# terryye/cuda_FlashAttention

Hardware: AMD Instinct MI355X
Metric: FA2 fwd+bwd TFLOP/s at (B=4,H=16,N=8192,d=128); % MFMA peak (higher is better)
Workload: dtype bf16; 1 GPU; FA2 forward+backward bf16, (B=4,H=16,N=8192,d=128) per GPU, non-causal (BASELINE configs[2]); flops = 14 B H N^2 d; B=4, H=16, N=8192, d=128, parallelism=head-sharded replicas x1

## Files before the change

### cuda_flashattention_amd/csrc/fa2_bwd_fused.hip

```cpp
#include <cstdlib>
#include <cstring>
#include <type_traits>

#include "fa2_regfile.h"
#include "fa2_launch.h"

namespace fa2 {

#include "fa2_bwd_fused_body.inc"

typedef __attribute__((address_space(3))) void* fused_lptr_t;

#ifndef FA2_FUSED_DSKEY
#define FA2_FUSED_DSKEY(row) (((row) >> 1) & 7)
#endif

#ifndef FA2_FUSED_DIAG
#define FA2_FUSED_DIAG 0
#endif

constexpr int kFusedRegFile = RF512;

#define FA2_FUSED_CLOBBERS "memory", "vcc", FA2_RF512
#define FA2_FUSED_OPS_128 [r0] "v"(roff[0]), [r1] "v"(roff[1]), [r2] "v"(roff[2]), [r3] "v"(roff[3]), [r4] "v"(roff[4]), [r5] "v"(roff[5]),  \
    [r6] "v"(roff[6]), [r7] "v"(roff[7]), [t0] "v"(toff[0]), [t1] "v"(toff[1]), [t2] "v"(toff[2]), [t3] "v"(toff[3]), [t4] "v"(toff[4]),   \
    [t5] "v"(toff[5]), [t6] "v"(toff[6]), [t7] "v"(toff[7]), [rc] "v"(rcv), [c2] "s"(c2)
#define FA2_FUSED_OPS_64 [r0] "v"(roff[0]), [r1] "v"(roff[1]), [r2] "v"(roff[2]), [r3] "v"(roff[3]), [t0] "v"(toff[0]), [t1] "v"(toff[1]),    \
    [t2] "v"(toff[2]), [t3] "v"(toff[3]), [rc] "v"(rcv), [c2] "s"(c2)

struct FusedStep {
    __amdgpu_buffer_rsrc_t drs, lrs, qrs, grs, rcrs, ctl;
    uint32_t dso, lso, qso, rcso, pvo, mso;
    int need, pval;
};
#define FA2_FUSED_STEP(TEXT, DD, ...)                                                                                                 \
    asm volatile(TEXT                                                                                                                 \
                 : [err] "+s"(err)                                                                                                    \
                 : FA2_FUSED_OPS_##DD, [vm] "i"(VMW), [dqv] "v"(dqv), [drs] "s"(f.drs), [dso] "s"(f.dso), [lrs] "s"(f.lrs), [lso] "s"(f.lso), \
                   [mw] "s"(mw), [mw2] "s"(mw2), [qrs] "s"(f.qrs), [grs] "s"(f.grs), [rcrs] "s"(f.rcrs), [qso] "s"(f.qso),               \
                   [rcso] "s"(f.rcso), [dvo] "v"(dvo), [rcvo] "v"(rcvo), [wv] "s"(wv), [ctl] "s"(f.ctl), [pvo] "s"(f.pvo),               \
                   [mso] "s"(f.mso), [need] "s"(f.need), [pval] "s"(f.pval) __VA_ARGS__                                                \
                 : FA2_FUSED_CLOBBERS, "s12", "s13", "scc", "exec", "m0", "v39")
template <int D, int BUF, int PAR, int VMW, bool MASKED>
__device__ __forceinline__ void fused_cbody(const uint32_t (&roff)[D / 16], const uint32_t (&toff)[D / 16], uint32_t rcv, float c2, uint32_t dqv,
                                            uint32_t dvo, uint32_t rcvo, uint32_t mw, uint32_t mw2, int wv, const FusedStep& f, int& err,
                                            int lo0 = 0, int lo1 = 0)
{
// ... 60 lines not shown

struct FusedArgs {
    BwdArgs b;
    float* dQacc;
    int* ctl;
    int npad;
    const float* rc;
    int fault;
};

#ifdef FA2_TEST_HOOKS
static int g_hook_fault = 0, g_hook_grid = 0, g_hook_last_grid = 0;
extern "C" void fa2_test_set_fused_hooks(int fault, int grid) { g_hook_fault = fault; g_hook_grid = grid; }
extern "C" int fa2_test_last_fused_grid(void) { return g_hook_last_grid; }
#define FA2_HOOK_NOTE_GRID(n) (g_hook_last_grid = (n))
#else
constexpr int g_hook_fault = 0, g_hook_grid = 0;
#define FA2_HOOK_NOTE_GRID(n) ((void)0)
#endif

__device__ __forceinline__ int fused_ctl_ints(int BH, int ncb) { return kCtlHeadmap + 16 * (BH + kHmPad) + 9 * BH * ncb; }

__device__ __forceinline__ int fused_load_sc1(const int* p)
{
    int v;
    asm volatile("global_load_dword %0, %1, off sc1\n\ts_waitcnt vmcnt(0)" : "=v"(v) : "v"(p) : "memory");
    return v;
}
__device__ __forceinline__ void fused_seen_set(int v)
{
    asm volatile("v_mov_b32 v39, %0" : : "s"(v) : "v39");
}

__device__ __forceinline__ int fused_lane_id() { return (int)__builtin_amdgcn_mbcnt_hi(~0u, __builtin_amdgcn_mbcnt_lo(~0u, 0u)); }
template <int OFF>
__device__ __forceinline__ int fused_mail_read(uint32_t lds_addr)
{
    int v;
    asm volatile("v_mov_b32 %0, %1\n\tds_read_b32 %0, %0 offset:%c2\n\ts_waitcnt lgkmcnt(0)" : "=&v"(v) : "s"(lds_addr), "i"(OFF) : "memory");
    return __builtin_amdgcn_readfirstlane(v);
}

__device__ __forceinline__ void fused_store_flag(int* p, int v)
{
    asm volatile("global_store_dword %0, %1, off" : : "v"(p), "v"(v) : "memory");
}

__device__ __forceinline__ bool fused_spin_over(int* ctl, int spins)
{
    if (spins > kSpinLimit) {
        atomicExch(ctl + kCtlError, 1);
        return true;
    }
    return (spins & 1023) == 0 && fused_load_sc1(ctl + kCtlError) != 0;
}

template <bool CHAIN, bool CAUSAL, bool RAGGED = false, bool RECT = false, int HD = 128>
__global__ void __launch_bounds__(256, 1) __attribute__((amdgpu_num_vgpr(39))) fa2_bwd_fused_kernel(FusedArgs fp)
{
    static_assert(CHAIN || !RAGGED, "the atomics form has no ragged variant");
    static_assert(!RECT || (CHAIN && !CAUSAL && !RAGGED), "rectangular blocks: chained, unmasked, aligned");
    static_assert(HD == 128 || (HD == 64 && CHAIN && !RECT), "head_dim 64: chained, square");
    extern __shared__ __attribute__((aligned(16))) char smem[];
    const BwdArgs& p = fp.b;
    constexpr int D = HD, ROWB = 2 * D, KS = D / 16, DT = D / 32;
    constexpr int DQW = 128;
    constexpr int TROWS = 32;
// ... 33 lines not shown
#pragma unroll
    for (int dt = 0; dt < DT; ++dt)
#pragma unroll
        for (int jj = 0; jj < 2; ++jj)
            toff[2 * dt + jj] = lbase + QRING + lds_off<D>(8 * jj + 4 * h + trq, 4 * dt + 2 * trcb + (trp >> 1)) + 8 * (trp & 1);
    const uint32_t rcv = lbase + QRING + 2 * TROWS * ROWB + 16 * h;
    static_for<KS>([&](auto S) {
        constexpr int sidx = decltype(S)::value;
        vset<kFusedRegFile, CL_TOP, ROFFK + sidx>(lbase + lds_off<D>(ki + 64 * wave, 2 * sidx + h));
    });
    const int ecol = W ? wave : (wave & 1), ekey0 = W ? 0 : 128 * (wave >> 1);
    static_for<2>([&](auto JJ) {
        constexpr int jj = decltype(JJ)::value;
        vset<kFusedRegFile, CL_TOP, KT + jj>(lbase + ekey0 * ROWB + lds_off<D>(8 * jj + 4 * h + trq, 4 * ecol + 2 * trcb + (trp >> 1)) + 8 * (trp & 1));
        const int row = 8 * jj + 4 * h + trq;
        vset<kFusedRegFile, CL_TOP, DSRD + jj>(lbase + DSB + (ekey0 + row) * 64 + 8 * ((4 * trcb + trp) ^ FA2_FUSED_DSKEY(row)));
    });
    static_for<4>([&](auto C) {
        constexpr int c = decltype(C)::value;
        vset<kFusedRegFile, CL_TOP, DSWR + c>(lbase + DSB + (64 * wave + ki) * 64 + 8 * (((2 * c) | h) ^ FA2_FUSED_DSKEY(ki)));
    });
    const int doff = lds_dma_off<D>(wave * RPI, lane);
    const uint32_t dqv = CHAIN ? (uint32_t)(wave * 4096 + lane * 16) : (uint32_t)(((4 * h) * D + 32 * wave + ki) * 4);
    const auto rc_rsrc = __builtin_amdgcn_make_buffer_rsrc((void*)fp.rc, 0, (int)(2 * rc_plane * 4), 0x00020000);

    int xcc = 0;
    if constexpr (CHAIN) {
        asm volatile("s_getreg_b32 %0, hwreg(HW_REG_XCC_ID, 0, 4)" : "=s"(xcc));
    }
    int* const prog_base = fp.ctl + kCtlHeadmap + 16 * (p.BH + kHmPad);
#ifndef FA2_FUSED_CAUSAL_G
#define FA2_FUSED_CAUSAL_G 2
#endif
    const int G = CAUSAL ? max(1, min(FA2_FUSED_CAUSAL_G, p.BH / 8)) : 1;
    const auto ctl_rsrc = __builtin_amdgcn_make_buffer_rsrc((void*)fp.ctl, 0, CHAIN ? fused_ctl_ints(p.BH, ncb) * 4 : 0, 0x00020000);

    auto take_ticket = [&]() {
        if (wave == 0 && fused_lane_id() == 0) {
            int hd, j = 0;
            do {
                const int u = atomicAdd(fp.ctl + kCtlTicket + 32 * xcc, 1);
                const int r = u % (G * ncb);
                const int k = (u / (G * ncb)) * G + r % G;
                j = r / G;
                hd = -2;
                if (k < p.BH + kHmPad) {
                    int* hm = fp.ctl + kCtlHeadmap + xcc * (p.BH + kHmPad) + k;
                    int v = 0, spins = 0;
                    if (j == 0) {
                        if (k > 0)
                            while ((v = fused_load_sc1(hm - 1)) == 0)
                                if (fused_spin_over(fp.ctl, ++spins)) break;
                        if (k > 0 && v == 0) {
                            v = -1;
                        } else {
                            const int g = atomicAdd(fp.ctl + kCtlNextHead, 1);
                            v = g < p.BH ? g + 1 : -1;
                        }
                        fused_store_flag(hm, v);
                    } else {
                        while ((v = fused_load_sc1(hm)) == 0)
                            if (fused_spin_over(fp.ctl, ++spins)) { v = -1; break; }
                    }
                    hd = v > 0 ? v - 1 : (r % G == 0 ? -2 : -1);
                }
            } while (hd == -1);
            mail[0] = hd;
            mail[1] = j;
            mail[2] = hd >= 0 ? fused_load_sc1(fp.ctl + kCtlError) : 0;
        }
    };
    auto issue_unit_loads = [&](int head_, int cb_) {
        const size_t slab_ = (size_t)(head_ / p.kv_group) * KHS * ROWB;
        const char* Kh_ = (const char*)p.K + slab_;
        const char* Vh_ = (const char*)p.V + slab_;
        const int kw0_ = cb_ * 256 + wave * 64;
        const int lane_u = (int)__builtin_amdgcn_mbcnt_hi(~0u, __builtin_amdgcn_mbcnt_lo(~0u, 0u));
        const int vk0 = RAGGED ? min(kw0_ + (lane_u & 31), N - 1) : kw0_ + (lane_u & 31);
        const int vk1 = RAGGED ? min(kw0_ + 32 + (lane_u & 31), N - 1) : kw0_ + 32 + (lane_u & 31);
        const char* v0 = Vh_ + (size_t)vk0 * ROWB + 16 * (lane_u >> 5);
        const char* v1 = Vh_ + (size_t)vk1 * ROWB + 16 * (lane_u >> 5);
        static_for<KS>([&](auto S) { fused_load_vfrag<VF, KS, decltype(S)::value>(v0, v1); });
        const auto k_rsrc = __builtin_amdgcn_make_buffer_rsrc((void*)Kh_, 0, N * ROWB, 0x00020000);
#pragma unroll
        for (int j = wave; j < 256 / RPI; j += 4)
            __builtin_amdgcn_raw_ptr_buffer_load_lds(k_rsrc, (fused_lptr_t)(smem + j * 1024), 16, doff, (cb_ * 256 + j * RPI) * ROWB, 0, FA2_FUSED_KV_AUX);
    };

    auto next_unit_loads = [&]() {
        if constexpr (CHAIN) {
            take_ticket();
            __syncthreads();
            const int hn = fused_mail_read<0>(mail_addr);
            if (hn >= 0) issue_unit_loads(hn, fused_mail_read<4>(mail_addr));
        }
    };
    next_unit_loads();

    for (;;) {
#ifdef FA2_FUSED_STATS
        const uint64_t s_pull = __builtin_readcyclecounter();
#endif
        int head, cb, err0 = 0;
        if constexpr (CHAIN) {
            head = fused_mail_read<0>(mail_addr);
            cb = fused_mail_read<4>(mail_addr);
            err0 = fused_mail_read<8>(mail_addr);
            if (head < 0) break;
        } else {
            map_block(blockIdx.x, p.BH, ncb, head, cb);
// ... 19 lines not shown
                const int soff = (t * TROWS + piece * RPI) * ROWB;
                __builtin_amdgcn_raw_ptr_buffer_load_lds(which ? g_rsrc : q_rsrc, (fused_lptr_t)(b + which * (TROWS * ROWB) + piece * 1024),
                                                         16, doff, soff, 0, 0);
            }
            if (wave < 2 && fused_lane_id() < 32)
                __builtin_amdgcn_raw_ptr_buffer_load_lds(rc_rsrc, (fused_lptr_t)(b + 2 * TROWS * ROWB + wave * 128), 4, rcoff, t * TROWS * 4, 0, 0);
        };
        const int n_u = CAUSAL ? ntiles - 8 * cb : ntiles;
        const int niter_u = CAUSAL ? ((n_u + 1 + 5) / 6) * 6 : niter;
        const bool ragged_unit = RAGGED && !CAUSAL && cb == ncb - 1;
        const int first_masked = CAUSAL ? ((n_u - 8) / 6) * 6 : (ragged_unit ? 0 : niter_u);
        auto tl = [&](int u) { return CAUSAL ? ntiles - 1 - u : u; };
        stage(tl(0), 0);
#ifdef FA2_FUSED_PREFILL
        stage(tl(1), 1);
        stage(tl(2), 2);
#endif
        fused_dq_zero<DQT>();
        asm volatile("s_waitcnt vmcnt(0)" ::: "memory");
        __syncthreads();
        if constexpr (W) asm volatile(FA2_FUSED_PRO : : FA2_FUSED_OPS_128, [vm] "i"(VMW) : FA2_FUSED_CLOBBERS);
        else asm volatile(FA2_FUSED64_PRO : : FA2_FUSED_OPS_64, [vm] "i"(VMW) : FA2_FUSED_CLOBBERS);

        const auto dq_rsrc = __builtin_amdgcn_make_buffer_rsrc((void*)(fp.dQacc + (size_t)head * NPQ * DQW), 0, NPQ * DQW * 4, 0x00020000);
        int* const mine = prog_base + head * ncb + cb;
        const int* const prev = mine - 1;
        const int prev_off = (int)((prev - fp.ctl) * 4);
        const int mine_off = (int)((mine - fp.ctl) * 4);
        if constexpr (CHAIN) fused_seen_set(0);
        int err = err0;
#ifdef FA2_FUSED_STATS
        int st_steps = 0, st_polls = 0, st_cycles = 0;
        const uint64_t u0 = __builtin_readcyclecounter();
#endif

        const auto null_rsrc = __builtin_amdgcn_make_buffer_rsrc((void*)fp.dQacc, 0, 0, 0x00020000);
        const bool hp_unit = cb > 0;
        const auto lrs_unit = hp_unit && !(FA2_FUSED_DIAG & 2) ? dq_rsrc : null_rsrc;
        auto step = [&](auto BUF, auto PAR, auto MASKED, auto FAST_, int t) {
            constexpr int buf = decltype(BUF)::value, par = decltype(PAR)::value;
            constexpr bool masked = decltype(MASKED)::value;
            constexpr bool FAST = decltype(FAST_)::value;
            if constexpr (CHAIN && FAST) {
                FusedStep f;
                f.drs = dq_rsrc;
                f.lrs = lrs_unit;
                f.dso = (uint32_t)(tl(t - 1) * TROWS * DQW * 4);
                f.lso = (uint32_t)(tl(t) * TROWS * DQW * 4);
                f.qrs = q_rsrc; f.grs = g_rsrc; f.rcrs = rc_rsrc; f.ctl = ctl_rsrc;
                f.qso = (uint32_t)(tl(t + 1) * TROWS * ROWB + wave * 1024);
                f.rcso = (uint32_t)(tl(t + 1) * TROWS * 4);
                f.pvo = (uint32_t)prev_off; f.mso = (uint32_t)mine_off;
                f.need = (hp_unit && !err && !(FA2_FUSED_DIAG & 1)) ? t + 1 : (int)0x80000000;
                f.pval = t;
#ifdef FA2_TEST_HOOKS
                if (fp.fault && cb == 1) f.pval = 0;
#endif
                fused_cbody<D, buf, par, VMW, false>(roff, toff, rcv, c2, dqv, (uint32_t)doff, (uint32_t)rcoff, lbase + QRING + wave * 1024,
                                                  lbase + QRING + wave * 128, wave, f, err, 0, 0);
            } else if constexpr (CHAIN) {
                FusedStep f;
                const bool live = t >= 1 && t <= n_u;
                const bool more = t + 1 < n_u;
                const bool has_prev = t < n_u && cb > 0;
                f.drs = live ? dq_rsrc : null_rsrc;
                f.lrs = has_prev && !(FA2_FUSED_DIAG & 2) ? dq_rsrc : null_rsrc;
                f.dso = (uint32_t)__builtin_amdgcn_readfirstlane(tl(t - 1) * TROWS * DQW * 4);
                f.lso = (uint32_t)__builtin_amdgcn_readfirstlane(tl(t) * TROWS * DQW * 4);
                f.qrs = q_rsrc; f.grs = g_rsrc; f.rcrs = rc_rsrc; f.ctl = ctl_rsrc;
                f.qso = more ? (uint32_t)(tl(t + 1) * TROWS * ROWB + wave * 1024) : 0x40000000u;
                f.rcso = more ? (uint32_t)(tl(t + 1) * TROWS * 4) : 0x40000000u;
                f.pvo = (uint32_t)prev_off; f.mso = (uint32_t)mine_off;
                f.need = (has_prev && !err && !(FA2_FUSED_DIAG & 1)) ? t + 1 : (int)0x80000000;
                f.pval = t < n_u ? t : n_u;
#ifdef FA2_TEST_HOOKS
                if (fp.fault && cb == 1) f.pval = 0;
#endif
                int lo0 = 0, lo1 = 0;
                if constexpr (masked) {
                    const int lane_m = (int)__builtin_amdgcn_mbcnt_hi(~0u, __builtin_amdgcn_mbcnt_lo(~0u, 0u));
                    if constexpr (CAUSAL) {
                        lo0 = kw0 + (lane_m & 31) - 4 * (lane_m >> 5) - TROWS * tl(t);
                        lo1 = lo0 + 32;
                    } else {
                        lo0 = kw0 + (lane_m & 31) < N ? -0x40000000 : 0x40000000;
                        lo1 = kw0 + 32 + (lane_m & 31) < N ? -0x40000000 : 0x40000000;
                    }
                }
#ifdef FA2_FUSED_STATS2
                const uint64_t b0 = __builtin_readcyclecounter();
#endif
                fused_cbody<D, buf, par, VMW, masked>(roff, toff, rcv, c2, dqv, (uint32_t)doff, (uint32_t)rcoff, lbase + QRING + wave * 1024,
                                                   lbase + QRING + wave * 128, wave, f, err, lo0, lo1);
#ifdef FA2_FUSED_STATS2
                st_cycles += (int)(__builtin_readcyclecounter() - b0);
#endif
            } else {
                static_assert(W || CHAIN, "head_dim 64: chained form only");
                stage(t + 1, (buf + 1) % 3);
                if constexpr (W) fused_body<buf, par, VMW>(roff, toff, rcv, c2);
#ifndef FA2_FUSED_NO_DQ
                if (t >= 1 && t <= ntiles) fused_dq_atomic<DQT>(dq_rsrc, dqv, (uint32_t)__builtin_amdgcn_readfirstlane((t - 1) * TROWS * D * 4));
#endif
                fused_dq_zero<DQT>();
            }
        };
        auto six = [&](auto MASKED, auto FAST_, int t) {
            step(std::integral_constant<int, 0>{}, std::integral_constant<int, 0>{}, MASKED, FAST_, t);
            step(std::integral_constant<int, 1>{}, std::integral_constant<int, 1>{}, MASKED, FAST_, t + 1);
            step(std::integral_constant<int, 2>{}, std::integral_constant<int, 0>{}, MASKED, FAST_, t + 2);
            step(std::integral_constant<int, 0>{}, std::integral_constant<int, 1>{}, MASKED, FAST_, t + 3);
            step(std::integral_constant<int, 1>{}, std::integral_constant<int, 0>{}, MASKED, FAST_, t + 4);
            step(std::integral_constant<int, 2>{}, std::integral_constant<int, 1>{}, MASKED, FAST_, t + 5);
        };
        const int fast_end = CHAIN ? n_u - 2 : -1;
        {
            const int plain_end = first_masked;
            int t = 0;
            asm volatile("" : "+s"(t));
            if (t < plain_end) { six(std::false_type{}, std::false_type{}, t); t += 6; }
#pragma unroll 1
            for (; t + 5 <= fast_end && t < plain_end; t += 6) six(std::false_type{}, std::true_type{}, t);
#pragma unroll 1
            for (; t < plain_end; t += 6) six(std::false_type{}, std::false_type{}, t);
            if constexpr (CHAIN && (CAUSAL || RAGGED)) {
#pragma unroll 1
                for (; t < niter_u; t += 6) six(std::true_type{}, std::false_type{}, t);
            }
        }
        asm volatile("s_waitcnt vmcnt(0) lgkmcnt(0)" ::: "memory");
        if constexpr (CHAIN)
            if (err && !err0 && wave == 0 && fused_lane_id() == 0) atomicExch(fp.ctl + kCtlError, 1);
#ifdef FA2_FUSED_STATS
        const uint64_t s_loop = __builtin_readcyclecounter();
#endif
        next_unit_loads();

        mfma_acc_settle();
        const int lane_ep = (int)__builtin_amdgcn_mbcnt_hi(~0u, __builtin_amdgcn_mbcnt_lo(~0u, 0u));
        const int ki_ep = lane_ep & 31, h_ep = lane_ep >> 5;
        static_for<2>([&](auto KB) {
            constexpr int kb = decltype(KB)::value;
            const int key = kw0 + 32 * kb + ki_ep;
            const size_t slab_k = RECT ? (size_t)head * KHS * ROWB : slab;
            char* const dKb = (char*)p.dK + slab_k;
            char* const dVb = (char*)p.dV + slab_k;
            const uint32_t koff = (uint32_t)key * ROWB + 16u * h_ep;
            char* dKk = dKb + koff;
            char* dVk = dVb + koff;
            static_for<2 * DT>([&](auto G) {
                constexpr int dt = decltype(G)::value / 2, gp = decltype(G)::value % 2;
                constexpr int RK = 16 * (kb * DT + dt) + 8 * gp, RV = 32 * DT + RK;
                auto pack4 = [&](float a, float b, float c, float d, float sc) {
                    bf16x4 v;
                    v[0] = (__bf16)(a * sc); v[1] = (__bf16)(b * sc); v[2] = (__bf16)(c * sc); v[3] = (__bf16)(d * sc);
                    return __builtin_bit_cast(u32x2, v);
                };
                auto emit = [&](u32x2 x, u32x2 y, char* dst) {
                    const auto s0 = __builtin_amdgcn_permlane32_swap(x[0], y[0], false, false);
                    const auto s1 = __builtin_amdgcn_permlane32_swap(x[1], y[1], false, false);
                    const u32x4 o = {s0[0], s1[0], s0[1], s1[1]};
#ifdef FA2_FUSED_ST_NT
                    if (!RAGGED || key < N) __builtin_nontemporal_store(o, reinterpret_cast<u32x4*>(dst + 2 * (32 * dt + 16 * gp)));
#else
                    if (!RAGGED || key < N) *reinterpret_cast<u32x4*>(dst + 2 * (32 * dt + 16 * gp)) = o;
#endif
                };
                emit(pack4(aread<RK>(), aread<RK + 1>(), aread<RK + 2>(), aread<RK + 3>(), p.scale),
                     pack4(aread<RK + 4>(), aread<RK + 5>(), aread<RK + 6>(), aread<RK + 7>(), p.scale), dKk);
                emit(pack4(aread<RV>(), aread<RV + 1>(), aread<RV + 2>(), aread<RV + 3>(), 1.0f),
                     pack4(aread<RV + 4>(), aread<RV + 5>(), aread<RV + 6>(), aread<RV + 7>(), 1.0f), dVk);
            });
        });
#ifdef FA2_FUSED_STATS
        if (CHAIN && wave == 0 && fused_lane_id() == 0) {
            atomicAdd(fp.ctl + kCtlError + 1, st_steps);
            atomicAdd(fp.ctl + kCtlError + 2, st_polls);
            atomicAdd((unsigned long long*)(fp.ctl + kCtlError + 4), (unsigned long long)st_cycles);
            atomicAdd((unsigned long long*)(fp.ctl + kCtlError + 6), (unsigned long long)(__builtin_readcyclecounter() - u0));
            int* rec = prog_base + p.BH * ncb + 8 * (head * ncb + cb);
            rec[0] = xcc; rec[1] = st_cycles; rec[2] = (int)(u0 - s_pull); rec[3] = (int)(__builtin_readcyclecounter() - s_loop);
            *(unsigned long long*)(rec + 4) = u0; *(unsigned long long*)(rec + 6) = __builtin_readcyclecounter();
        }
#endif
        if constexpr (!CHAIN) break;
    }
}

__global__ void __launch_bounds__(256) fa2_bwd_fused_dq_out_kernel(const float* __restrict__ acc, __bf16* __restrict__ dQ, size_t n8, float scale,
                                                                    const int* __restrict__ err)
{
    const float poison = (err && *err) ? __builtin_nanf("") : 0.0f;
    const size_t stride = (size_t)gridDim.x * 256;
    for (size_t i = (size_t)blockIdx.x * 256 + threadIdx.x; i < n8; i += stride) {
        const f32x4 a = reinterpret_cast<const f32x4*>(acc)[2 * i], b = reinterpret_cast<const f32x4*>(acc)[2 * i + 1];
        bf16x8 o;
#pragma unroll
        for (int e = 0; e < 4; ++e) { o[e] = (__bf16)(a[e] * scale + poison); o[4 + e] = (__bf16)(b[e] * scale + poison); }
        reinterpret_cast<bf16x8*>(dQ)[i] = o;
    }
}

__global__ void __launch_bounds__(256) fa2_bwd_fused_dq_out_chain_kernel(const float* __restrict__ acc, __bf16* __restrict__ dQ, size_t n4, float scale,
                                                                          const int* __restrict__ err, int N, int NP, int qhs)
{
    const float poison = *err ? __builtin_nanf("") : 0.0f;
    const size_t stride = (size_t)gridDim.x * 256;
    const size_t tiles = (size_t)(NP / 32);
    for (size_t i = (size_t)blockIdx.x * 256 + threadIdx.x; i < n4; i += stride) {
        const f32x4 a = reinterpret_cast<const f32x4*>(acc)[i];
        const int lane = (int)(i & 63), g = (int)((i >> 6) & 3), wave = (int)((i >> 8) & 3);
        const size_t tg = i >> 10, head = tg / tiles;
        const int row = (int)(tg % tiles) * 32 + 8 * g + 4 * (lane >> 5);
        __bf16* o = dQ + (head * (size_t)qhs + row) * 128 + 32 * wave + (lane & 31);
#pragma unroll
// ... 182 lines not shown
```

### cuda_flashattention_amd/csrc/fa2_common.h

```cpp
#pragma once
#include <hip/hip_runtime.h>
#include <stdint.h>

#include <type_traits>
#include <utility>

namespace fa2 {

typedef __attribute__((ext_vector_type(8))) __bf16 bf16x8;
typedef __attribute__((ext_vector_type(4))) __bf16 bf16x4;
typedef __attribute__((ext_vector_type(16))) float f32x16;
typedef __attribute__((ext_vector_type(4))) float f32x4;
typedef __attribute__((ext_vector_type(2))) float f32x2;
typedef __attribute__((ext_vector_type(4))) uint32_t u32x4;
typedef __attribute__((ext_vector_type(2))) uint32_t u32x2;

constexpr float kLog2e = 1.4426950408889634f;

template <int D>
__device__ __forceinline__ int lds_off(int row, int ch)
{
    static_assert(D == 64 || D == 128, "head_dim must be 64 or 128");
    if constexpr (D == 128)
        return 256 * row + 16 * (ch ^ (((row & 3) << 2) | ((row >> 2) & 3)));
    else
        return 128 * row + 16 * (ch ^ ((((row >> 1) & 1) << 2) | ((row >> 2) & 3)));
}

template <int D>
__device__ __forceinline__ int lds_dma_off(int row0, int lane)
{
    constexpr int ROWB = 2 * D, CPR = D / 8;
    const int drow = lane / CPR, dslot = lane % CPR, prow = row0 + drow;
    return drow * ROWB + 16 * ((lds_off<D>(prow, dslot) - ROWB * prow) >> 4);
}

template <typename F, int... I>
__device__ __forceinline__ void static_for_impl(F&& f, std::integer_sequence<int, I...>)
{
    (f(std::integral_constant<int, I>{}), ...);
}
template <int N, typename F>
__device__ __forceinline__ void static_for(F&& f)
{
    static_for_impl(f, std::make_integer_sequence<int, N>{});
}

__device__ __forceinline__ float half_max(float x)
{
    const uint32_t u = __float_as_uint(x);
    auto r = __builtin_amdgcn_permlane32_swap(u, u, false, false);
    return fmaxf(__uint_as_float(r[0]), __uint_as_float(r[1]));
}

__device__ __forceinline__ float half_sum(float x)
{
    const uint32_t u = __float_as_uint(x);
    auto r = __builtin_amdgcn_permlane32_swap(u, u, false, false);
    return __uint_as_float(r[0]) + __uint_as_float(r[1]);
}

__device__ __forceinline__ constexpr int acc_row(int r, int h)
{
    return (r & 3) + 8 * (r >> 2) + 4 * h;
}

__device__ __forceinline__ void map_block(int bid, int n_heads, int nrb, int& head, int& rb)
// ... 26 lines not shown
```

### cuda_flashattention_amd/csrc/fa2_fwd1_bf16.hip

```cpp
#include <type_traits>

#include "fa2_fwd_softmax.h"
#include "fa2_launch.h"

namespace fa2 {

#include "fa2_fwd_body.inc"

constexpr int kF1Rows = 256;
constexpr int kF1Bufs = 4;
constexpr float kF1SumLimit = 1.2089258e24f;
constexpr float kF1LiftAt = 1.0737418e9f;
constexpr float kF1LiftBy = 44.3614196f;
enum { F1_PLAIN = 0, F1_MASKED = 1, F1_NOMAX = 2 };

typedef __attribute__((address_space(3))) void* f1_lptr_t;

template <int QBS> constexpr int kF1RegFile = QBS == 2 ? RF512 : RF128;

struct F1Dma {
    __amdgpu_buffer_rsrc_t krs, vrs;
    uint32_t mw, dvo, kso;
};

template <int D, int QBS, int BUF, int KB, int MODE>
__device__ __forceinline__ void f1_body(float c2, int& need, const int (&hi)[2], const F1Dma& dma)
{
#define FA2_F1_CASE(TAG, DD, QQ, B, K, MV, M)                                                                                      \
    if constexpr (D == DD && QBS == QQ && BUF == B && KB == K && MODE == MV)                                                         \
        FA2_RF_ASM(kF1RegFile<QQ>, CL_ORDER, FA2_FWD_BODY_##TAG##_B##B##_K##K##_##M, [need] "=&s"(need),                                                     \
                   [c2] "s"(c2) FA2_COMMA [hi0] "v"(hi[0]) FA2_COMMA [hi1] "v"(hi[1]) FA2_COMMA [ninf] "v"(-INFINITY)           \
                       FA2_COMMA [mw] "s"(dma.mw) FA2_COMMA [dvo] "v"(dma.dvo) FA2_COMMA [krs] "s"(dma.krs)                     \
                       FA2_COMMA [vrs] "s"(dma.vrs) FA2_COMMA [kso] "s"(dma.kso));
#define FA2_F1_CASES_B(TAG, DD, QQ, K, MV, M) \
    FA2_F1_CASE(TAG, DD, QQ, 0, K, MV, M) FA2_F1_CASE(TAG, DD, QQ, 1, K, MV, M) FA2_F1_CASE(TAG, DD, QQ, 2, K, MV, M) FA2_F1_CASE(TAG, DD, QQ, 3, K, MV, M)
#define FA2_F1_CASES_V(TAG, DD, QQ, K) \
    FA2_F1_CASES_B(TAG, DD, QQ, K, F1_PLAIN, M0) FA2_F1_CASES_B(TAG, DD, QQ, K, F1_MASKED, M1) FA2_F1_CASES_B(TAG, DD, QQ, K, F1_NOMAX, X)
    FA2_F1_CASES_V(D128Q2, 128, 2, 0) FA2_F1_CASES_V(D128Q2, 128, 2, 1)
    FA2_F1_CASES_V(D64Q2, 64, 2, 0) FA2_F1_CASES_V(D64Q2, 64, 2, 1) FA2_F1_CASES_V(D64Q2, 64, 2, 2) FA2_F1_CASES_V(D64Q2, 64, 2, 3)
    FA2_F1_CASES_V(D64Q1, 64, 1, 0) FA2_F1_CASES_V(D64Q1, 64, 1, 1) FA2_F1_CASES_V(D64Q1, 64, 1, 2) FA2_F1_CASES_V(D64Q1, 64, 1, 3)
#undef FA2_F1_CASES_V
#undef FA2_F1_CASES_B
#undef FA2_F1_CASE
}

template <int D, int QBS>
__device__ __forceinline__ void f1_prologue()
{
    if constexpr (D == 128) FA2_RF_ASM(RF512, CL_ORDER, FA2_FWD_PRO_D128Q2, , );
// ... 227 lines not shown
            constexpr int kb = decltype(KB_)::value;
            const int j = t * NH + kb;
            int need = 0;
            if constexpr (GENERAL) {
                if (j >= JB) return;
                const int key0 = j * 32;
                bool masked = key0 + 32 > Nk;
                if (CAUSAL) masked = masked || key0 + 31 > q0 + p.causal_shift;
                if (masked) {
                    int hi[2] = {0, 0};
#pragma unroll
                    for (int qb = 0; qb < QBS; ++qb) hi[qb] = (CAUSAL ? min(Nk, qrow[qb] + p.causal_shift + 1) : Nk) - key0 - 4 * h;
                    f1_body<D, QBS, B, kb, F1_MASKED>(c2, need, hi, dma);
                } else {
                    const int hi[2] = {0, 0};
                    f1_body<D, QBS, B, kb, F1_PLAIN>(c2, need, hi, dma);
                }
            } else {
                const int hi[2] = {0, 0};
                f1_body<D, QBS, B, kb, FAST>(c2, need, hi, dma);
            }
            if (__builtin_amdgcn_readfirstlane(need | (int)have_pend)) update(need);
        });
    };
    const int ntl = (JB + NH - 1) / NH;
    int nfull = Nk / KV;
    if (CAUSAL) nfull = min(nfull, max(0, (q0 + p.causal_shift + 1) / KV));
    nfull = min(nfull, J / NH) & ~3;
    int nfull_wg = Nk / KV;
    if (CAUSAL) nfull_wg = min(nfull_wg, max(0, (rb * kF1Rows + (kF1Waves - 1) * WROWS + p.causal_shift + 1) / KV));
    nfull_wg = min(nfull_wg, J / NH) & ~3;
    using I0 = Int<0>; using I1 = Int<1>; using I2 = Int<2>; using I3 = Int<3>;
    int* const redo_flag = reinterpret_cast<int*>(smem + 2 * KRING);
    bool safe = false;
    for (;;) {
        init_pass();
        out_of_range = false;
        asm volatile("s_waitcnt vmcnt(0)" ::: "memory");
        __syncthreads();
        f1_prologue<D, QBS>();
        int t = 0;
        for (; t < nfull; t += 4) {
            if (safe) {
                run_tile(I0{}, I0{}, t); run_tile(I1{}, I0{}, t + 1); run_tile(I2{}, I0{}, t + 2); run_tile(I3{}, I0{}, t + 3);
            } else if (t == 0) {
                run_tile(I0{}, I0{}, t); run_tile(I1{}, I2{}, t + 1); run_tile(I2{}, I2{}, t + 2); run_tile(I3{}, I2{}, t + 3);
            } else {
                lift();
                run_tile(I0{}, I2{}, t); run_tile(I1{}, I2{}, t + 1); run_tile(I2{}, I2{}, t + 2); run_tile(I3{}, I2{}, t + 3);
            }
        }
        FA2_FWD_TAIL_TILES(run_tile, t, ntl);
        asm volatile("s_waitcnt vmcnt(0) lgkmcnt(0)" ::: "memory");
        if (safe || nfull_wg == 0) break;
        bool bad = out_of_range;
        static_for<QBS>([&](auto QB) {
            constexpr int qb = decltype(QB)::value;
            bad = bad || !(half_sum(vget<ST + 2 * qb>() + vget<ST + 2 * qb + 1>()) < kF1SumLimit);
        });
        if (tid == 0) *redo_flag = 0;
        __syncthreads();
        if (__any(bad) && lane == 0) *redo_flag = 1;
        __syncthreads();
        if (*redo_flag == 0) break;
        asm volatile("; fa2-cold: a row sum left the range of the rounds without maxima: the row block again, with maxima");
        safe = true;
    }
    mfma_acc_settle();
    const bool fin = !STATE || p.finalize;
    static_for<QBS>([&](auto QB) {
        constexpr int qb = decltype(QB)::value;
        const float l_tot = half_sum(vget<ST + 2 * qb>() + vget<ST + 2 * qb + 1>());
        const size_t qoff = (size_t)head * qhs + qrow[qb];
        const float pa = pend[qb];
        const float inv = (fin ? (l_tot > 0.0f ? 1.0f / l_tot : 0.0f) : 1.0f) * pa;
        static_for<2 * DT>([&](auto G) {
            constexpr int dt = decltype(G)::value / 2, gp = decltype(G)::value % 2;
            constexpr int R = A_O + (qb * DT + dt) * 16 + 8 * gp;
            f32x4 v, w;
            fwd_read_o8<R>(inv, v, w);
            if (fin) {
                const u32x4 o = fwd_pack_o8_bf16(v, w);
                if (qrow[qb] < Nq) *reinterpret_cast<u32x4*>((char*)p.O + qoff * ROWB + 2 * (32 * dt + 16 * gp + 8 * h)) = o;
            } else if (qrow[qb] < Nq) {
                *reinterpret_cast<f32x4*>(p.Oacc + qoff * D + 32 * dt + 16 * gp + 4 * h) = v;
                *reinterpret_cast<f32x4*>(p.Oacc + qoff * D + 32 * dt + 16 * gp + 8 + 4 * h) = w;
            }
        });
        if (qrow[qb] < Nq && h == 0) {
            if (fin) {
                p.L[qoff] = m_run[qb] + __builtin_logf(l_tot);
            } else {
                p.L[qoff] = l_tot;
                p.M[qoff] = m_run[qb];
            }
        }
    });
    }
}

template <int D, int QBS, bool CAUSAL, bool STATE>
__device__ __forceinline__ void fwd1_dense_impl(const FwdArgs& p)
{
    const int nrb = (p.Nq + kF1Rows - 1) / kF1Rows;
    const int nwg = (CAUSAL && !STATE) ? (nrb + 1) / 2 : nrb;
    int head, wi;
    map_block(blockIdx.x, p.BH, nwg, head, wi);
    fa2_fwd1_impl<D, QBS, CAUSAL, STATE>(p, head, wi);
}

template <int D, int QBS, bool CAUSAL>
__device__ __forceinline__ void fwd1_varlen_impl(const VarlenFwdArgs& v)
{
    constexpr size_t ROWB = D * 2;
    int head, idx;
    map_block(blockIdx.x, v.a.BH, v.n_items, head, idx);
    const VarlenItem it = uniform_item(v.items, idx);
    FwdArgs p = v.a;
    p.Q = (const char*)p.Q + (size_t)it.q_row0 * ROWB;
    p.O = (char*)p.O + (size_t)it.q_row0 * ROWB;
    p.L += it.q_row0;
    p.K = (const char*)p.K + (size_t)it.k_row0 * ROWB;
    p.V = (const char*)p.V + (size_t)it.k_row0 * ROWB;
    p.Nq = it.len_q; p.Nk = it.len_k;
    p.resume = 0; p.finalize = 1;
    const int nrb = (it.len_q + kF1Rows - 1) / kF1Rows;
    fa2_fwd1_impl<D, QBS, CAUSAL, true>(p, head, CAUSAL ? nrb - 1 - it.block : it.block);
}

template <int D, bool CAUSAL, bool STATE>
// ... 70 lines not shown
```

Measured before the change: 1341 TFLOP/s.

## Stage dK/dV epilogue through LDS for row-contiguous stores; group dense tickets

New measurement: 1320 TFLOP/s. -1.6%, worse.

```diff
diff --git a/cuda_flashattention_amd/csrc/fa2_bwd_fused.hip b/cuda_flashattention_amd/csrc/fa2_bwd_fused.hip
--- a/cuda_flashattention_amd/csrc/fa2_bwd_fused.hip
+++ b/cuda_flashattention_amd/csrc/fa2_bwd_fused.hip
@@ -10,9 +10,20 @@
 #include "fa2_bwd_fused_body.inc"
 
 typedef __attribute__((address_space(3))) void* fused_lptr_t;
+typedef __attribute__((address_space(1))) u32x4 fused_gvec_t;
 
 #ifndef FA2_FUSED_DSKEY
 #define FA2_FUSED_DSKEY(row) (((row) >> 1) & 7)
+#endif
+
+#ifndef FA2_FUSED_ROWST
+#define FA2_FUSED_ROWST 1
+#endif
+#ifndef FA2_FUSED_ROWST_NG
+#define FA2_FUSED_ROWST_NG 2
+#endif
+#ifndef FA2_FUSED_DENSE_G
+#define FA2_FUSED_DENSE_G 2
 #endif
 
 #ifndef FA2_FUSED_DIAG
@@ -239,7 +250,8 @@
 #ifndef FA2_FUSED_CAUSAL_G
 #define FA2_FUSED_CAUSAL_G 2
 #endif
-    const int G = CAUSAL ? max(1, min(FA2_FUSED_CAUSAL_G, p.BH / 8)) : 1;
+    const int G = CAUSAL ? max(1, min(FA2_FUSED_CAUSAL_G, p.BH / 8))
+                         : ((FA2_FUSED_DENSE_G > 1 && CHAIN && !RECT) ? max(1, min(FA2_FUSED_DENSE_G, p.BH / 8)) : 1);
     const auto ctl_rsrc = __builtin_amdgcn_make_buffer_rsrc((void*)fp.ctl, 0, CHAIN ? fused_ctl_ints(p.BH, ncb) * 4 : 0, 0x00020000);
 
     auto take_ticket = [&]() {
@@ -473,6 +485,71 @@
         next_unit_loads();
 
         mfma_acc_settle();
+#if FA2_FUSED_ROWST
+        if constexpr (!CHAIN) __syncthreads();
+        auto lane_fresh = [&]() {
+            int l;
+            asm volatile("v_mbcnt_lo_u32_b32 %0, -1, 0\n\tv_mbcnt_hi_u32_b32 %0, -1, %0" : "=v"(l));
+            return l;
+        };
+        static_for<4>([&](auto B) {
+            constexpr int kb = decltype(B)::value / 2;
+            constexpr bool isv = decltype(B)::value % 2;
+            constexpr int CPRW = ROWB / 16, RPS = 1024 / ROWB;
+            char* const stg = smem + DSB + wave * 8192;
+            const float sc = isv ? 1.0f : p.scale;
+            {
+                const int lw = lane_fresh(), kiw = lw & 31;
+                char* const wrow = stg + kiw * ROWB;
+                const int cw = (lw >> 5) ^ (kiw & 7);
+                static_for<2 * DT>([&](auto G) {
+                    constexpr int dt = decltype(G)::value / 2, gp = decltype(G)::value % 2;
+                    constexpr int R0 = (isv ? 32 * DT : 0) + 16 * (kb * DT + dt) + 8 * gp;
+                    auto pack2 = [&](float a, float b) {
+                        typedef float pair_f32 __attribute__((ext_vector_type(2)));
+                        typedef __bf16 pair_bf16 __attribute__((ext_vector_type(2)));
+                        const pair_f32 v = {a * sc, b * sc};
+                        return __builtin_bit_cast(uint32_t, __builtin_convertvector(v, pair_bf16));
+                    };
+                    auto pack4 = [&](float a, float b, float c, float d) { return u32x2{pack2(a, b), pack2(c, d)}; };
+                    const u32x2 x = pack4(aread<R0>(), aread<R0 + 1>(), aread<R0 + 2>(), aread<R0 + 3>());
+                    const u32x2 y = pack4(aread<R0 + 4>(), aread<R0 + 5>(), aread<R0 + 6>(), aread<R0 + 7>());
+                    const auto s0 = __builtin_amdgcn_permlane32_swap(x[0], y[0], false, false);
+                    const auto s1 = __builtin_amdgcn_permlane32_swap(x[1], y[1], false, false);
+                    const u32x4 o = {s0[0], s1[0], s0[1], s1[1]};
+                    *reinterpret_cast<u32x4*>(wrow + 16 * (cw ^ (4 * dt + 2 * gp))) = o;
+                    __builtin_amdgcn_sched_barrier(0);
+                });
+            }
+            const int key0 = kw0 + 32 * kb;
+            const size_t slab_k = RECT ? (size_t)head * KHS * ROWB : slab;
+            char* const dst = (char*)(isv ? p.dV : p.dK) + slab_k + (size_t)key0 * ROWB;
+            const uint32_t lr = (uint32_t)lane_fresh();
+            const uint32_t loff = 16u * lr;
+            const int rr = (int)(lr / CPRW), cc = (int)(lr % CPRW);
+            constexpr int NG = (W && (CAUSAL || RAGGED)) ? 1 : FA2_FUSED_ROWST_NG;
+            static_for<32 / RPS / NG>([&](auto GR) {
+                constexpr int i0 = decltype(GR)::value * NG;
+                uintptr_t gb = (uintptr_t)dst + 1024 * i0;
+                asm volatile("" : "+s"(gb));
+                u32x4 o[NG];
+                static_for<NG>([&](auto I) {
+                    const int row = RPS * (i0 + decltype(I)::value) + rr;
+                    o[decltype(I)::value] = *reinterpret_cast<const u32x4*>(stg + row * ROWB + 16 * (cc ^ (row & 7)));
+                });
+                static_for<NG>([&](auto I) {
+                    constexpr int i = decltype(I)::value;
+                    const int left = min(N - key0 - RPS * (i0 + i), 32);
+#ifdef FA2_FUSED_ST_NT
+                    if (!RAGGED || (int)loff < left * ROWB) __builtin_nontemporal_store(o[i], (fused_gvec_t*)(gb + (uint32_t)(loff + 1024 * i)));
+#else
+                    if (!RAGGED || (int)loff < left * ROWB) *(fused_gvec_t*)(gb + (uint32_t)(loff + 1024 * i)) = o[i];
+#endif
+                });
+                __builtin_amdgcn_sched_barrier(0);
+            });
+        });
+#else
         const int lane_ep = (int)__builtin_amdgcn_mbcnt_hi(~0u, __builtin_amdgcn_mbcnt_lo(~0u, 0u));
         const int ki_ep = lane_ep & 31, h_ep = lane_ep >> 5;
         static_for<2>([&](auto KB) {
@@ -508,6 +585,7 @@
                      pack4(aread<RV + 4>(), aread<RV + 5>(), aread<RV + 6>(), aread<RV + 7>(), 1.0f), dVk);
             });
         });
+#endif
 #ifdef FA2_FUSED_STATS
         if (CHAIN && wave == 0 && fused_lane_id() == 0) {
             atomicAdd(fp.ctl + kCtlError + 1, st_steps);
```

## Stage dK/dV and O epilogue stores through swizzled LDS for row-contiguous global writes

Applied to the files above, without the earlier changes.

Result: no change. 1276 TFLOP/s before, 1273 TFLOP/s after (-0.2%).

```diff
diff --git a/cuda_flashattention_amd/csrc/fa2_bwd_fused.hip b/cuda_flashattention_amd/csrc/fa2_bwd_fused.hip
--- a/cuda_flashattention_amd/csrc/fa2_bwd_fused.hip
+++ b/cuda_flashattention_amd/csrc/fa2_bwd_fused.hip
@@ -139,7 +139,12 @@
     asm volatile("v_mov_b32 v39, %0" : : "s"(v) : "v39");
 }
 
-__device__ __forceinline__ int fused_lane_id() { return (int)__builtin_amdgcn_mbcnt_hi(~0u, __builtin_amdgcn_mbcnt_lo(~0u, 0u)); }
+__device__ __forceinline__ int fused_lane_id()
+{
+    int l;
+    asm volatile("v_mbcnt_lo_u32_b32 %0, -1, 0\n\tv_mbcnt_hi_u32_b32 %0, -1, %0" : "=v"(l));
+    return l;
+}
 template <int OFF>
 __device__ __forceinline__ int fused_mail_read(uint32_t lds_addr)
 {
@@ -239,16 +244,19 @@
 #ifndef FA2_FUSED_CAUSAL_G
 #define FA2_FUSED_CAUSAL_G 2
 #endif
-    const int G = CAUSAL ? max(1, min(FA2_FUSED_CAUSAL_G, p.BH / 8)) : 1;
+    auto group_of = [](int heads) { return CAUSAL ? max(1, min(FA2_FUSED_CAUSAL_G, heads / 8)) : 1; };
     const auto ctl_rsrc = __builtin_amdgcn_make_buffer_rsrc((void*)fp.ctl, 0, CHAIN ? fused_ctl_ints(p.BH, ncb) * 4 : 0, 0x00020000);
 
     auto take_ticket = [&]() {
         if (wave == 0 && fused_lane_id() == 0) {
             int hd, j = 0;
+            int heads = p.BH, nkb = ncb;
+            asm volatile("" : "+s"(heads), "+s"(nkb));
+            const int G = group_of(heads), gn = G * nkb;
             do {
                 const int u = atomicAdd(fp.ctl + kCtlTicket + 32 * xcc, 1);
-                const int r = u % (G * ncb);
-                const int k = (u / (G * ncb)) * G + r % G;
+                const int r = u % gn;
+                const int k = (u / gn) * G + r % G;
                 j = r / G;
                 hd = -2;
                 if (k < p.BH + kHmPad) {
@@ -282,7 +290,7 @@
         const char* Kh_ = (const char*)p.K + slab_;
         const char* Vh_ = (const char*)p.V + slab_;
         const int kw0_ = cb_ * 256 + wave * 64;
-        const int lane_u = (int)__builtin_amdgcn_mbcnt_hi(~0u, __builtin_amdgcn_mbcnt_lo(~0u, 0u));
+        const int lane_u = fused_lane_id();
         const int vk0 = RAGGED ? min(kw0_ + (lane_u & 31), N - 1) : kw0_ + (lane_u & 31);
         const int vk1 = RAGGED ? min(kw0_ + 32 + (lane_u & 31), N - 1) : kw0_ + 32 + (lane_u & 31);
         const char* v0 = Vh_ + (size_t)vk0 * ROWB + 16 * (lane_u >> 5);
@@ -368,6 +376,7 @@
 #ifdef FA2_FUSED_STATS
         int st_steps = 0, st_polls = 0, st_cycles = 0;
         const uint64_t u0 = __builtin_readcyclecounter();
+        uint64_t s_two = u0;
 #endif
 
         const auto null_rsrc = __builtin_amdgcn_make_buffer_rsrc((void*)fp.dQacc, 0, 0, 0x00020000);
@@ -414,7 +423,7 @@
 #endif
                 int lo0 = 0, lo1 = 0;
                 if constexpr (masked) {
-                    const int lane_m = (int)__builtin_amdgcn_mbcnt_hi(~0u, __builtin_amdgcn_mbcnt_lo(~0u, 0u));
+                    const int lane_m = fused_lane_id();
                     if constexpr (CAUSAL) {
                         lo0 = kw0 + (lane_m & 31) - 4 * (lane_m >> 5) - TROWS * tl(t);
                         lo1 = lo0 + 32;
@@ -430,6 +439,9 @@
                                                    lbase + QRING + wave * 128, wave, f, err, lo0, lo1);
 #ifdef FA2_FUSED_STATS2
                 st_cycles += (int)(__builtin_readcyclecounter() - b0);
+#endif
+#ifdef FA2_FUSED_STATS
+                if (t == 1) s_two = __builtin_readcyclecounter();
 #endif
             } else {
                 static_assert(W || CHAIN, "head_dim 64: chained form only");
@@ -471,42 +483,76 @@
         const uint64_t s_loop = __builtin_readcyclecounter();
 #endif
         next_unit_loads();
+#ifdef FA2_FUSED_STATS
+        const uint64_t s_next = __builtin_readcyclecounter();
+#endif
 
         mfma_acc_settle();
-        const int lane_ep = (int)__builtin_amdgcn_mbcnt_hi(~0u, __builtin_amdgcn_mbcnt_lo(~0u, 0u));
+        const int lane_ep = fused_lane_id();
         const int ki_ep = lane_ep & 31, h_ep = lane_ep >> 5;
+        static_assert(32 * ROWB <= 2 * (FA2_FUSED_DSTILE / 4) && FA2_FUSED_DSTILE == FA2_FUSED64_DSTILE, "the wave's rows of the two dS tiles hold a block");
+        constexpr int DSWAVE = FA2_FUSED_DSTILE / 4;
+        constexpr int HOP = FA2_FUSED_DSTILE - DSWAVE;
+        constexpr int EPI_PER = W ? 2 : 1;
+        static_assert(epi_read_periodic<D, EPI_PER>(), "the rows of reads i and i + EPI_PER have the same swizzle key");
+        const uint32_t img = lbase + DSB + wave * DSWAVE;
+        const uint32_t wrow = img + ROWB * ki_ep + (W ? (ki_ep >> 4) * HOP : 0);
+        uint32_t wkey = 16 * (h_ep ^ (ki_ep & 7));
+        uint32_t rd[EPI_PER];
+#pragma unroll
+        for (int k = 0; k < EPI_PER; ++k) rd[k] = img + epi_read_off<D>(lane_ep, k) - 1024 * k;
         static_for<2>([&](auto KB) {
             constexpr int kb = decltype(KB)::value;
-            const int key = kw0 + 32 * kb + ki_ep;
+            const int key0 = kw0 + 32 * kb;
             const size_t slab_k = RECT ? (size_t)head * KHS * ROWB : slab;
-            char* const dKb = (char*)p.dK + slab_k;
-            char* const dVb = (char*)p.dV + slab_k;
-            const uint32_t koff = (uint32_t)key * ROWB + 16u * h_ep;
-            char* dKk = dKb + koff;
-            char* dVk = dVb + koff;
+            char* const dKb = (char*)p.dK + slab_k + (size_t)key0 * ROWB;
+            char* const dVb = (char*)p.dV + slab_k + (size_t)key0 * ROWB;
+            auto pack4 = [&](float a, float b, float c, float d, float sc) {
+                bf16x4 v;
+                v[0] = (__bf16)(a * sc); v[1] = (__bf16)(b * sc); v[2] = (__bf16)(c * sc); v[3] = (__bf16)(d * sc);
+                return __builtin_bit_cast(u32x2, v);
+            };
+            auto put = [&](u32x2 x, u32x2 y, int g, char* dst) {
+                if (g == 0) asm volatile("" : "+v"(wkey));
+
+                const auto s0 = __builtin_amdgcn_permlane32_swap(x[0], y[0], false, false);
+                const auto s1 = __builtin_amdgcn_permlane32_swap(x[1], y[1], false, false);
+                const u32x4 o = {s0[0], s1[0], s0[1], s1[1]};
+#ifdef FA2_FUSED_EPI_DIRECT
+                if (!RAGGED || key0 + ki_ep < N) *reinterpret_cast<u32x4*>(dst + (uint32_t)ki_ep * ROWB + 32 * g + 16 * h_ep) = o;
+#else
+                *lds_ptr16(wrow + (wkey ^ (32 * g))) = o;
+#endif
+            };
+            auto rows_out = [&](char* dst) {
+#ifndef FA2_FUSED_EPI_DIRECT
+                static_for<NINS>([&](auto I) {
+                    constexpr int i = decltype(I)::value;
+                    const u32x4 o = *lds_ptr16(rd[i % EPI_PER] + 1024 * i + (1024 * i >= DSWAVE ? HOP : 0));
+                    char* const at = dst + 1024 * i + (uint32_t)(16 * lane_ep);
+                    if (!RAGGED || key0 + RPI * i + lane_ep / CPR < N) {
+#ifdef FA2_FUSED_ST_NT
+                        __builtin_nontemporal_store(o, reinterpret_cast<u32x4*>(at));
+#else
+                        *reinterpret_cast<u32x4*>(at) = o;
+#endif
+                    }
+                    if constexpr (i % 2 == 1) asm volatile("" ::: "memory");
+                });
+#endif
+            };
             static_for<2 * DT>([&](auto G) {
-                constexpr int dt = decltype(G)::value / 2, gp = decltype(G)::value % 2;
-                constexpr int RK = 16 * (kb * DT + dt) + 8 * gp, RV = 32 * DT + RK;
-                auto pack4 = [&](float a, float b, float c, float d, float sc) {
-                    bf16x4 v;
-                    v[0] = (__bf16)(a * sc); v[1] = (__bf16)(b * sc); v[2] = (__bf16)(c * sc); v[3] = (__bf16)(d * sc);
-                    return __builtin_bit_cast(u32x2, v);
-                };
-                auto emit = [&](u32x2 x, u32x2 y, char* dst) {
-                    const auto s0 = __builtin_amdgcn_permlane32_swap(x[0], y[0], false, false);
-                    const auto s1 = __builtin_amdgcn_permlane32_swap(x[1], y[1], false, false);
-                    const u32x4 o = {s0[0], s1[0], s0[1], s1[1]};
-#ifdef FA2_FUSED_ST_NT
-                    if (!RAGGED || key < N) __builtin_nontemporal_store(o, reinterpret_cast<u32x4*>(dst + 2 * (32 * dt + 16 * gp)));
-#else
-                    if (!RAGGED || key < N) *reinterpret_cast<u32x4*>(dst + 2 * (32 * dt + 16 * gp)) = o;
-#endif
-                };
-                emit(pack4(aread<RK>(), aread<RK + 1>(), aread<RK + 2>(), aread<RK + 3>(), p.scale),
-                     pack4(aread<RK + 4>(), aread<RK + 5>(), aread<RK + 6>(), aread<RK + 7>(), p.scale), dKk);
-                emit(pack4(aread<RV>(), aread<RV + 1>(), aread<RV + 2>(), aread<RV + 3>(), 1.0f),
-                     pack4(aread<RV + 4>(), aread<RV + 5>(), aread<RV + 6>(), aread<RV + 7>(), 1.0f), dVk);
+                constexpr int g = decltype(G)::value, RK = 16 * kb * DT + 8 * g;
+                put(pack4(aread<RK>(), aread<RK + 1>(), aread<RK + 2>(), aread<RK + 3>(), p.scale),
+                    pack4(aread<RK + 4>(), aread<RK + 5>(), aread<RK + 6>(), aread<RK + 7>(), p.scale), g, dKb);
             });
+            rows_out(dKb);
+            static_for<2 * DT>([&](auto G) {
+                constexpr int g = decltype(G)::value, RV = 32 * DT + 16 * kb * DT + 8 * g;
+                put(pack4(aread<RV>(), aread<RV + 1>(), aread<RV + 2>(), aread<RV + 3>(), 1.0f),
+                    pack4(aread<RV + 4>(), aread<RV + 5>(), aread<RV + 6>(), aread<RV + 7>(), 1.0f), g, dVb);
+            });
+            rows_out(dVb);
         });
 #ifdef FA2_FUSED_STATS
         if (CHAIN && wave == 0 && fused_lane_id() == 0) {
@@ -515,8 +561,14 @@
             atomicAdd((unsigned long long*)(fp.ctl + kCtlError + 4), (unsigned long long)st_cycles);
             atomicAdd((unsigned long long*)(fp.ctl + kCtlError + 6), (unsigned long long)(__builtin_readcyclecounter() - u0));
             int* rec = prog_base + p.BH * ncb + 8 * (head * ncb + cb);
-            rec[0] = xcc; rec[1] = st_cycles; rec[2] = (int)(u0 - s_pull); rec[3] = (int)(__builtin_readcyclecounter() - s_loop);
-            *(unsigned long long*)(rec + 4) = u0; *(unsigned long long*)(rec + 6) = __builtin_readcyclecounter();
+            rec[0] = xcc;
+#ifdef FA2_FUSED_STATS2
+            rec[1] = st_cycles;
+#else
+            rec[1] = (int)(s_next - s_loop);
+#endif
+            rec[2] = (int)(u0 - s_pull); rec[3] = (int)(__builtin_readcyclecounter() - s_loop);
+            *(unsigned long long*)(rec + 4) = u0; rec[6] = (int)(__builtin_readcyclecounter() - u0); rec[7] = (int)(s_two - u0);
         }
 #endif
         if constexpr (!CHAIN) break;
diff --git a/cuda_flashattention_amd/csrc/fa2_common.h b/cuda_flashattention_amd/csrc/fa2_common.h
--- a/cuda_flashattention_amd/csrc/fa2_common.h
+++ b/cuda_flashattention_amd/csrc/fa2_common.h
@@ -33,6 +33,28 @@
     constexpr int ROWB = 2 * D, CPR = D / 8;
     const int drow = lane / CPR, dslot = lane % CPR, prow = row0 + drow;
     return drow * ROWB + 16 * ((lds_off<D>(prow, dslot) - ROWB * prow) >> 4);
+}
+
+template <int D>
+__device__ __forceinline__ constexpr int epi_off(int row, int pc)
+{
+    static_assert(D == 64 || D == 128, "head_dim must be 64 or 128");
+    return 2 * D * row + 16 * (pc ^ (row & 7));
+}
+template <int D>
+__device__ __forceinline__ constexpr int epi_read_off(int lane, int i)
+{
+    return epi_off<D>(lane / (D / 8) + (512 / D) * i, lane % (D / 8));
+}
+typedef __attribute__((address_space(3))) u32x4 lds_u32x4;
+__device__ __forceinline__ lds_u32x4* lds_ptr16(uint32_t addr) { return reinterpret_cast<lds_u32x4*>((uintptr_t)addr); }
+template <int D, int PER>
+constexpr bool epi_read_periodic()
+{
+    for (int l = 0; l < 64; ++l)
+        for (int i = 0; i < D / 16; ++i)
+            if (epi_read_off<D>(l, i) != epi_read_off<D>(l, i % PER) + 1024 * (i - i % PER)) return false;
+    return true;
 }
 
 template <typename F, int... I>
diff --git a/cuda_flashattention_amd/csrc/fa2_fwd1_bf16.hip b/cuda_flashattention_amd/csrc/fa2_fwd1_bf16.hip
--- a/cuda_flashattention_amd/csrc/fa2_fwd1_bf16.hip
+++ b/cuda_flashattention_amd/csrc/fa2_fwd1_bf16.hip
@@ -15,6 +15,22 @@
 enum { F1_PLAIN = 0, F1_MASKED = 1, F1_NOMAX = 2 };
 
 typedef __attribute__((address_space(3))) void* f1_lptr_t;
+
+#ifdef FA2_F1_EPI_STAMPS
+constexpr unsigned kF1StampSlots = 1u << 16;
+__device__ unsigned g_f1_stamps[4 * kF1StampSlots];
+extern "C" __attribute__((visibility("default"))) int fa2_debug_read_fwd_stamps(unsigned* host, int clear)
+{
+    hipError_t e = hipDeviceSynchronize();
+    if (e == hipSuccess) e = hipMemcpyFromSymbol(host, HIP_SYMBOL(g_f1_stamps), sizeof(unsigned) * 4 * kF1StampSlots);
+    if (e == hipSuccess && clear) {
+        void* dev = nullptr;
+        e = hipGetSymbolAddress(&dev, HIP_SYMBOL(g_f1_stamps));
+        if (e == hipSuccess) e = hipMemset(dev, 0, sizeof(unsigned) * 4 * kF1StampSlots);
+    }
+    return (int)e;
+}
+#endif
 
 template <int QBS> constexpr int kF1RegFile = QBS == 2 ? RF512 : RF128;
 
@@ -308,6 +324,10 @@
     nfull_wg = min(nfull_wg, J / NH) & ~3;
     using I0 = Int<0>; using I1 = Int<1>; using I2 = Int<2>; using I3 = Int<3>;
     int* const redo_flag = reinterpret_cast<int*>(smem + 2 * KRING);
+    const bool fin = !STATE || p.finalize;
+#ifdef FA2_F1_EPI_STAMPS
+    const uint64_t s_wg = __builtin_readcyclecounter();
+#endif
     bool safe = false;
     for (;;) {
         init_pass();
@@ -328,7 +348,10 @@
         }
         FA2_FWD_TAIL_TILES(run_tile, t, ntl);
         asm volatile("s_waitcnt vmcnt(0) lgkmcnt(0)" ::: "memory");
-        if (safe || nfull_wg == 0) break;
+        if (safe || nfull_wg == 0) {
+            if (fin) __syncthreads();
+            break;
+        }
         bool bad = out_of_range;
         static_for<QBS>([&](auto QB) {
             constexpr int qb = decltype(QB)::value;
@@ -342,8 +365,20 @@
         asm volatile("; fa2-cold: a row sum left the range of the rounds without maxima: the row block again, with maxima");
         safe = true;
     }
+#ifdef FA2_F1_EPI_STAMPS
+    const uint64_t s_loop = __builtin_readcyclecounter();
+#endif
     mfma_acc_settle();
-    const bool fin = !STATE || p.finalize;
+    static_assert(kF1Rows * ROWB <= KRING, "the K ring holds the workgroup's rows of O");
+    constexpr int EPI_PER = D == 128 ? 2 : 1;
+    static_assert(epi_read_periodic<D, EPI_PER>(), "the rows of reads i and i + EPI_PER have the same swizzle key");
+    int lane_e = lane;
+    asm volatile("" : "+v"(lane_e));
+    const uint32_t img = lbase + wave * QBS * 32 * ROWB;
+    const uint32_t wrow = img + ROWB * (lane_e & 31), wkey = 16 * ((lane_e >> 5) ^ (lane_e & 7));
+    uint32_t rd[EPI_PER];
+#pragma unroll
+    for (int k = 0; k < EPI_PER; ++k) rd[k] = img + epi_read_off<D>(lane_e, k) - 1024 * k;
     static_for<QBS>([&](auto QB) {
         constexpr int qb = decltype(QB)::value;
         const float l_tot = half_sum(vget<ST + 2 * qb>() + vget<ST + 2 * qb + 1>());
@@ -351,18 +386,33 @@
         const float pa = pend[qb];
         const float inv = (fin ? (l_tot > 0.0f ? 1.0f / l_tot : 0.0f) : 1.0f) * pa;
         static_for<2 * DT>([&](auto G) {
-            constexpr int dt = decltype(G)::value / 2, gp = decltype(G)::value % 2;
+            constexpr int g = decltype(G)::value, dt = g / 2, gp = g % 2;
             constexpr int R = A_O + (qb * DT + dt) * 16 + 8 * gp;
             f32x4 v, w;
             fwd_read_o8<R>(inv, v, w);
             if (fin) {
                 const u32x4 o = fwd_pack_o8_bf16(v, w);
+#ifdef FA2_F1_EPI_DIRECT
                 if (qrow[qb] < Nq) *reinterpret_cast<u32x4*>((char*)p.O + qoff * ROWB + 2 * (32 * dt + 16 * gp + 8 * h)) = o;
+#else
+                *lds_ptr16(wrow + qb * 32 * ROWB + (wkey ^ (32 * g))) = o;
+#endif
             } else if (qrow[qb] < Nq) {
                 *reinterpret_cast<f32x4*>(p.Oacc + qoff * D + 32 * dt + 16 * gp + 4 * h) = v;
                 *reinterpret_cast<f32x4*>(p.Oacc + qoff * D + 32 * dt + 16 * gp + 8 + 4 * h) = w;
             }
         });
+#ifndef FA2_F1_EPI_DIRECT
+        if (fin) {
+            const int row0 = q0 + 32 * qb;
+            char* const dst = (char*)p.O + ((size_t)head * qhs + row0) * ROWB + (uint32_t)(16 * lane_e);
+            static_for<32 / RPI>([&](auto I) {
+                constexpr int i = decltype(I)::value;
+                const u32x4 o = *lds_ptr16(rd[i % EPI_PER] + qb * 32 * ROWB + 1024 * i);
+                if (row0 + RPI * i + lane_e / CPR < Nq) *reinterpret_cast<u32x4*>(dst + 1024 * i) = o;
+            });
+        }
+#endif
         if (qrow[qb] < Nq && h == 0) {
             if (fin) {
                 p.L[qoff] = m_run[qb] + __builtin_logf(l_tot);
@@ -372,6 +422,20 @@
             }
         }
     });
+#ifdef FA2_F1_EPI_STAMPS
+    {
+        const uint64_t s_iss = __builtin_readcyclecounter();
+        asm volatile("s_waitcnt vmcnt(0)" ::: "memory");
+        const uint64_t s_end = __builtin_readcyclecounter();
+        const unsigned slot = (blockIdx.x * kF1Waves + wave) * (PAIRED ? 2 : 1) + half;
+        if (lane == 0 && slot < kF1StampSlots) {
+            g_f1_stamps[4 * slot] = (unsigned)(s_loop - s_wg);
+            g_f1_stamps[4 * slot + 1] = (unsigned)(s_iss - s_loop);
+            g_f1_stamps[4 * slot + 2] = (unsigned)(s_end - s_loop);
+            g_f1_stamps[4 * slot + 3] = 1u;
+        }
+    }
+#endif
     }
 }
 
```
